# RozDavid/UnScene3D

Measured on AMD Instinct MI355X. Metric: training scenes/sec (Res16UNet34C+Mask3D, 150k voxels), higher is better.
Workload: dtype f32

## Files before the change

unscene3d_amd/csrc/common.h:

```cpp
#pragma once
#include <hip/hip_runtime.h>
#include <stdint.h>
#include <stdio.h>
#include <string.h>

#include "../../include/usc3d.h"

namespace usc {

constexpr int kWave = 64;

void set_error(const char* fmt, ...);

#define USC_REQUIRE(cond, ...)                   \
  do {                                           \
    if (!(cond)) {                               \
      ::usc::set_error(__VA_ARGS__);             \
      return USC_ERR_ARG;                        \
    }                                            \
  } while (0)

#define USC_CHECK_LAUNCH(name)                                                  \
  do {                                                                          \
    hipError_t e__ = hipGetLastError();                                         \
// ... 37 lines not shown
  k ^= k >> 31;
  return k;
}

__host__ __device__ inline int floor_quant(int c, int q) {
  int d = c / q;
  if ((c % q != 0) && ((c < 0) != (q < 0))) --d;
  return d * q;
}

#if defined(__HIPCC__)
__device__ inline int table_lookup(const uint64_t* __restrict__ keys,
                                   const int32_t* __restrict__ vals, int64_t cap,
                                   uint64_t key) {
  uint64_t slot = hash_key(key) & (uint64_t)(cap - 1);
  for (;;) {
    uint64_t k = keys[slot];
    if (k == key) return vals[slot];
    if (k == kEmptyKey) return -1;
    slot = (slot + 1) & (uint64_t)(cap - 1);
  }
}

__device__ inline int lane_id() { return threadIdx.x & 63; }

__device__ inline int wave_reduce_add(int v) {
#pragma unroll
  for (int o = 32; o > 0; o >>= 1) v += __shfl_xor(v, o, 64);
  return v;
}
__device__ inline float wave_reduce_addf(float v) {
#pragma unroll
  for (int o = 32; o > 0; o >>= 1) v += __shfl_xor(v, o, 64);
  return v;
}
__device__ inline double wave_reduce_addd(double v) {
#pragma unroll
  for (int o = 32; o > 0; o >>= 1) v += __shfl_xor(v, o, 64);
  return v;
}
__device__ inline int wave_inclusive_scan(int v) {
  const int l = lane_id();
#pragma unroll
  for (int o = 1; o < 64; o <<= 1) {
    int t = __shfl_up(v, o, 64);
    if (l >= o) v += t;
  }
  return v;
}
#endif

int spconv_up_table(const int32_t* nbr2, int32_t K, int64_t n_coarse, int64_t n_fine, int32_t* inv, hipStream_t st);

}
```

unscene3d_amd/csrc/spconv.hip:

```cpp
#include "common.h"

#include <stdlib.h>

#include <vector>

namespace usc {

typedef float f32x16 __attribute__((ext_vector_type(16)));

#define MFMA32(a, b, c) __builtin_amdgcn_mfma_f32_32x32x2f32((a), (b), (c), 0, 0, 0)

struct GemmParams {
  const float* in;
  const float* W;
  const int32_t* nbr;
  const float* bias;
  float* out;
  int64_t n_out;
  int cin, cout, K;
  int accumulate;
  int G;
  int TM;
  int wt1;
  const int32_t* rows_in;
  const int32_t* rows_out;
  const int64_t* koff;
  unsigned long long* stats;
};

__device__ inline int acc_row(int reg, int half) { return (reg & 3) + 8 * (reg >> 2) + 4 * half; }

template <int NB> struct BVec;
template <> struct BVec<1> { float v[1]; };
template <> struct BVec<2> { float v[2]; };
template <> struct BVec<3> { float v[3]; };
template <> struct BVec<4> { float v[4]; };

template <int NB>
__device__ inline void load_b(const float* __restrict__ p, float (&b)[NB]) {
  if (NB == 4) {
    const float4 t = *reinterpret_cast<const float4*>(p);
    b[0] = t.x; b[1 % NB] = t.y; b[2 % NB] = t.z; b[3 % NB] = t.w;
  } else if (NB == 2) {
    const float2 t = *reinterpret_cast<const float2*>(p);
    b[0] = t.x; b[1 % NB] = t.y;
  } else {
#pragma unroll
    for (int nb = 0; nb < NB; ++nb) b[nb] = p[nb];
  }
}

template <bool LIST>
__device__ inline bool locate_tile(const GemmParams& p, int wave, int i, int& k_begin, int& k_end,
                                   int64_t& my_out_row, int64_t& my_in_row_list) {
  my_out_row = -1;
  my_in_row_list = -1;
// ... 968 lines not shown
  pl.aligned = true;
  const int cb = cout / 32;
  const int cands[4] = {4, 3, 2, 1};
  int chosen = 1;
  for (int c = 0; c < 4; ++c) {
    const int nb = cands[c];
    if (cb % nb) continue;
    if (max_tiles * (cb / nb) >= kTargetWaves) { chosen = nb; break; }
  }
  pl.NB = chosen;
  return pl;
}

template <bool LIST>
static void launch_gemm(const GemmPlan& pl, dim3 grid, hipStream_t st, const GemmParams& p) {
#define USC_GG(NBv)                                                                                      \
  if (pl.aligned && p.wt1)        \
    hipLaunchKernelGGL((gather_gemm_aligned_kernel<NBv, false, true>), grid, dim3(256), 0, st, p);      \
  else if (pl.aligned)                                                                                   \
    hipLaunchKernelGGL((gather_gemm_aligned_kernel<NBv, LIST>), grid, dim3(256), 0, st, p);             \
  else                                                                                                   \
    hipLaunchKernelGGL((gather_gemm_kernel<NBv, LIST>), grid, dim3(256), 0, st, p);
  switch (pl.NB) {
    case 1: USC_GG(1) break;
    case 2: USC_GG(2) break;
    case 3: USC_GG(3) break;
    default: USC_GG(4) break;
  }
#undef USC_GG
}

}

using namespace usc;

extern "C" {

int usc_weight_transpose(const float* W, int32_t K, int32_t cin, int32_t cout, int32_t mirror, float* out,
                         usc_stream_t s) {
  USC_REQUIRE(W && out && K >= 1 && cin >= 1 && cout >= 1, "usc_weight_transpose: bad argument");
  const int64_t total = (int64_t)K * cin * cout;
  hipLaunchKernelGGL(weight_transpose_kernel, dim3(stream_grid(total, 256)), dim3(256), 0, as_stream(s), W, (int)K,
                     (int)cin, (int)cout, (int)mirror, out);
  USC_CHECK_LAUNCH("usc_weight_transpose");
  return USC_OK;
}

int usc_spconv_plan(int32_t kind, int64_t n, int32_t cin, int32_t cout, int32_t K) {
  GemmPlan pl;
  if (kind == 0 && stem_form(K > 1, cin, cout, K)) return 1 | (1 << 14);
  if (kind == 0) pl = plan_table(n, cin, cout, K);
  else if (kind == 1) pl = plan_list(ceil_div(n, 32) + K, cin, cout);
  else {
    const int ctiles = cin / 32, cb = cout / 32;
    const int NBf = (cb % 3 == 0) ? 3 : (cb % 4 == 0 ? 4 : (cb % 2 == 0 ? 2 : 1));
    if (cin % 32 == 0 && cout % 32 == 0 && (!(NBf == 3 && ctiles % 3 != 0) || ctiles % 4 == 0)) {
      const int CT = wgrad_full_ct(ctiles, NBf);
      return NBf | (1 << 8) | (1 << 13) | (CT << 16);
    }
    const int NB = pick_nb(cout);
    pl = GemmPlan{NB, 1, (cin % 32 == 0) && (cout % (NB * 32) == 0), 0};
  }
  return pl.NB | ((pl.aligned ? 1 : 0) << 8) | ((pl.TM > 0 ? 1 : 0) << 12) | (pl.G << 16);
}

int64_t usc_spconv_gather_gemm_ws_bytes(int64_t n_out, int32_t cin, int32_t cout, int32_t K) {
  const GemmPlan pl = plan_table(n_out, cin, cout, K);
  if (pl.TM > 0) return (int64_t)K * cin * cout * 4;
  return pl.G > 1 ? (int64_t)pl.G * n_out * cout * 4 : 0;
}

namespace {
struct LaunchStats { unsigned long long* ring = nullptr; int64_t slots = 0, count = 0; std::vector<usc_launch_stat> meta; };
LaunchStats g_lstats;
__global__ void launch_stats_init_kernel(unsigned long long* ring, int64_t slots) {
  const int64_t i = (int64_t)blockIdx.x * blockDim.x + threadIdx.x;
  if (i < slots) { ring[4 * i] = ~0ull; ring[4 * i + 1] = 0; ring[4 * i + 2] = 0; ring[4 * i + 3] = 0; }
}
}

int usc_launch_stats_begin(void* ring_dev, int64_t slots, usc_stream_t s) {
  USC_REQUIRE(ring_dev && slots > 0, "usc_launch_stats_begin: needs a device ring of slots x 4 x u64");
  hipLaunchKernelGGL(launch_stats_init_kernel, dim3((unsigned)ceil_div(slots, 256)), dim3(256), 0, as_stream(s),
                     (unsigned long long*)ring_dev, slots);
  USC_CHECK_LAUNCH("usc_launch_stats_begin");
  g_lstats.ring = (unsigned long long*)ring_dev;
  g_lstats.slots = slots;
  g_lstats.count = 0;
  g_lstats.meta.clear();
  g_lstats.meta.reserve((size_t)slots);
  return USC_OK;
}

int64_t usc_launch_stats_end(usc_launch_stat* host_out, int64_t max_out) {
  const int64_t n = g_lstats.count;
  if (host_out)
    for (int64_t i = 0; i < n && i < max_out; ++i) host_out[i] = g_lstats.meta[(size_t)i];
  g_lstats.ring = nullptr;
  g_lstats.slots = g_lstats.count = 0;
  g_lstats.meta.clear();
  return n;
}

int64_t usc_wall_clock_khz(void) {
  int dev = 0, khz = 0;
  if (hipGetDevice(&dev) != hipSuccess || hipDeviceGetAttribute(&khz, hipDeviceAttributeWallClockRate, dev) != hipSuccess) return 0;
  return khz;
}

int usc_spconv_gather_gemm(const float* in, int64_t n_in, int32_t cin, const float* W, int32_t K, int32_t cout,
                           const int32_t* nbr, int64_t n_out, const float* bias, float* out, int32_t accumulate,
                           int32_t w_transposed, void* ws, int64_t ws_bytes, usc_stream_t s) {
  USC_REQUIRE(cin >= 1 && cout >= 1 && K >= 1 && n_out >= 0 && n_in >= 0, "usc_spconv_gather_gemm: bad sizes");
  USC_REQUIRE(nbr || K == 1, "usc_spconv_gather_gemm: K>1 needs a neighbour table");
  USC_REQUIRE(nbr || n_in == n_out, "usc_spconv_gather_gemm: identity map needs n_in == n_out");
  if (n_out == 0) return USC_OK;
  USC_REQUIRE(in && W && out, "usc_spconv_gather_gemm: null pointer");
  if (stem_form(nbr != nullptr, cin, cout, K) && !accumulate && !w_transposed) {
    hipLaunchKernelGGL(stem_conv_kernel, dim3((unsigned)ceil_div(n_out, 256)), dim3(256), 0, as_stream(s), in, W, nbr, bias,
                       out, n_out, (int)K, (int)cin);
    USC_CHECK_LAUNCH("usc_spconv_gather_gemm");
    return USC_OK;
  }
  const GemmPlan pl = plan_table(n_out, cin, cout, K);
  GemmParams p{};
  p.in = in; p.W = W; p.nbr = nbr; p.bias = bias; p.out = out;
  p.n_out = n_out; p.cin = cin; p.cout = cout; p.K = K; p.accumulate = accumulate; p.G = pl.G;
  if (pl.G > 1) {
    USC_REQUIRE(ws && ws_bytes >= (int64_t)pl.G * n_out * cout * 4, "usc_spconv_gather_gemm: workspace too small");
    p.out = (float*)ws;
  }
  hipStream_t st = as_stream(s);
  const bool wt1 = w_transposed && K == 1 && !nbr && pl.aligned && pl.TM == 0;
  USC_REQUIRE(!w_transposed || pl.TM > 0 || wt1,
              "usc_spconv_gather_gemm: w_transposed is only folded into the tile-compacted kernel (usc_spconv_plan bit 12) "
              "and, for K = 1 on identity rows with channel counts in multiples of 32, into the row-order kernel; "
              "use usc_weight_transpose for other shapes");
  p.wt1 = wt1 ? 1 : 0;
  if (pl.TM > 0) {
    p.TM = pl.TM;
    USC_REQUIRE(ws && ws_bytes >= (int64_t)K * cin * cout * 4, "usc_spconv_gather_gemm: workspace too small");
    hipLaunchKernelGGL(weight_pack_kernel, dim3(stream_grid((int64_t)K * cin * cout, 256)), dim3(256), 0, st, W, (int)K,
                       (int)cin, (int)cout, pl.NB, (int)w_transposed, (float*)ws);
    p.W = (const float*)ws;
    dim3 cgrid((unsigned)ceil_div(n_out, pl.TM), (unsigned)(cout / (pl.NB * 32)));
    const size_t lds = compact_lds_bytes(pl.NB, pl.TM);
    if (g_lstats.ring && g_lstats.count < g_lstats.slots) {
      p.stats = g_lstats.ring + 4 * g_lstats.count++;
      g_lstats.meta.push_back(usc_launch_stat{n_out, cin, cout, K, pl.NB});
    }
#define USC_CG(NBv)                                                                                        \
    {                                                                                                      \
      static bool attr_set = false;                                                                        \
      auto kfn = gather_gemm_compact_kernel<NBv>;                                                          \
      if (!attr_set) {                                                                                     \
        (void)hipFuncSetAttribute((const void*)kfn, hipFuncAttributeMaxDynamicSharedMemorySize, 160 * 1024); \
        attr_set = true;                                                                                   \
      }                                                                                                    \
      hipLaunchKernelGGL(kfn, cgrid, dim3(64 * kCompactWaves), lds, st, p);                                \
    }
    if (pl.NB == 3) USC_CG(3) else if (pl.NB == 2) USC_CG(2) else USC_CG(1)
#undef USC_CG
    USC_CHECK_LAUNCH("usc_spconv_gather_gemm");
    return USC_OK;
  }
  dim3 grid((unsigned)ceil_div(n_out, 128), (unsigned)ceil_div(cout, pl.NB * 32), (unsigned)pl.G);
  launch_gemm<false>(pl, grid, st, p);
  if (pl.G > 1) {
    const int64_t numel4 = n_out * cout / 4;
    hipLaunchKernelGGL(group_reduce_kernel, dim3(stream_grid(numel4, 256)), dim3(256), 0, st, (const float*)ws, pl.G,
                       numel4, (int)cout, bias, (int)accumulate, out);
  }
  USC_CHECK_LAUNCH("usc_spconv_gather_gemm");
  return USC_OK;
}

int usc_spconv_pairs_gemm(const float* in, int32_t cin, const float* W, int32_t K, int32_t cout,
                          const int32_t* rows_in, const int32_t* rows_out, const int64_t* koff, int64_t P_capacity,
                          float* out, usc_stream_t s) {
  USC_REQUIRE(cin >= 1 && cout >= 1 && K >= 1 && P_capacity >= 0, "usc_spconv_pairs_gemm: bad sizes");
  if (P_capacity == 0) return USC_OK;
  USC_REQUIRE(in && W && rows_in && rows_out && koff && out, "usc_spconv_pairs_gemm: null pointer");
  GemmParams p{};
  p.in = in; p.W = W; p.out = out; p.cin = cin; p.cout = cout; p.K = K; p.G = 1;
  p.rows_in = rows_in; p.rows_out = rows_out; p.koff = koff;
  const int64_t max_tiles = ceil_div(P_capacity, 32) + K;
  const GemmPlan pl = plan_list(max_tiles, cin, cout);
  dim3 grid((unsigned)ceil_div(max_tiles, 4), (unsigned)ceil_div(cout, pl.NB * 32));
  launch_gemm<true>(pl, grid, as_stream(s), p);
  USC_CHECK_LAUNCH("usc_spconv_pairs_gemm");
  return USC_OK;
}

int64_t usc_spconv_wgrad_ws_bytes(int32_t K, int32_t cin, int32_t cout) {
  return (int64_t)64 * K * cin * cout * (int64_t)sizeof(float);
}

int64_t usc_spconv_wgrad_ws_bytes_rows(int32_t K, int32_t cin, int32_t cout, int64_t n_rows) {
  const int64_t numel = (int64_t)K * cin * cout;
  const int ctiles = cin / 32, cb = cout / 32;
  if (cin % 32 == 0 && cout % 32 == 0 && cb > 0) {
    const int NBf = wgrad_full_nb(cb);
    if (!(NBf == 3 && ctiles % 3 != 0) || ctiles % 4 == 0)
      return wgrad_full_splits(K, ctiles, cb, wgrad_full_ct(ctiles, NBf), NBf, n_rows) * numel * 4;
  }
  return (int64_t)wgrad_splits(K, cin, cout, pick_nb(cout), n_rows) * numel * 4;
}

int64_t usc_spconv_wgrad_table_ws_bytes(int32_t K, int32_t cin, int32_t cout) {
  return (int64_t)kStemSplits * K * cin * cout * 4;
}

int usc_spconv_wgrad_table(const float* in, int32_t cin, const float* dy, int32_t cout, const int32_t* nbr, int32_t K,
                           int64_t n_out, float* dW, int32_t accumulate, void* ws, int64_t ws_bytes, usc_stream_t s) {
  USC_REQUIRE(cin >= 1 && cin <= 4 && cout == 32 && K >= 1 && K <= 32 && n_out >= 0,
              "usc_spconv_wgrad_table: the table form covers <= 4 input channels and 32 output channels (the stem)");
  USC_REQUIRE(in && dy && nbr && dW && ws, "usc_spconv_wgrad_table: null pointer");
  USC_REQUIRE(ws_bytes >= usc_spconv_wgrad_table_ws_bytes(K, cin, cout), "usc_spconv_wgrad_table: workspace too small");
  hipStream_t st = as_stream(s);
  const int per = 32 / cin, groups = (K + per - 1) / per;
  const int64_t numel = (int64_t)K * cin * 32;
  hipLaunchKernelGGL(stem_wgrad_kernel, dim3(kStemSplits, (unsigned)groups), dim3(64 * kStemWaves), 0, st, in, dy, nbr, n_out, (int)K,
                     (int)cin, (float*)ws);
  hipLaunchKernelGGL(wgrad_reduce_kernel, dim3(stream_grid(numel, 256)), dim3(256), 0, st, (const float*)ws, kStemSplits, numel,
                     (int)accumulate, dW);
  USC_CHECK_LAUNCH("usc_spconv_wgrad_table");
  return USC_OK;
}

static int g_wgrad_grid_limit = 0;
void usc_spconv_wgrad_grid_limit(int32_t max_workgroups) { g_wgrad_grid_limit = max_workgroups; }

int usc_spconv_wgrad(const float* a, int32_t cin, const float* b, int32_t cout, int32_t K, const int32_t* a_idx,
                     const int32_t* b_idx, const int64_t* koff, int64_t n_rows, float* dW, int32_t accumulate, void* ws, int64_t ws_bytes,
                     usc_stream_t s) {
  USC_REQUIRE(cin >= 1 && cout >= 1 && K >= 1 && n_rows >= 0, "usc_spconv_wgrad: bad sizes");
  USC_REQUIRE(a && b && dW && ws, "usc_spconv_wgrad: null pointer");
  USC_REQUIRE((a_idx && b_idx && koff) || (!a_idx && K == 1), "usc_spconv_wgrad: pair lists required for K>1");
  const int64_t numel = (int64_t)K * cin * cout;
  hipStream_t st = as_stream(s);
  WgradParams p{};
  p.a = a; p.b = b; p.a_idx = a_idx; p.b_idx = b_idx; p.koff = koff; p.n_rows = n_rows;
  p.partial = (float*)ws; p.cin = cin; p.cout = cout; p.K = K;
  const int ctiles = cin / 32, cb = cout / 32;
  const int NBf = wgrad_full_nb(cb);
  if (cin % 32 == 0 && cout % 32 == 0 && (!(NBf == 3 && ctiles % 3 != 0) || ctiles % 4 == 0)) {
    const int CT = wgrad_full_ct(ctiles, NBf);
    const int64_t S = wgrad_full_splits(K, ctiles, cb, CT, NBf, n_rows);
    USC_REQUIRE(ws_bytes >= S * numel * 4, "usc_spconv_wgrad: workspace too small");
    p.S = (int)S;
    if (S == 1) { p.direct = dW; p.accumulate = accumulate; }
    dim3 grid((unsigned)(K * S), (unsigned)(ctiles / CT), (unsigned)(cb / NBf));
    if (g_wgrad_grid_limit > 0 && (int64_t)K * S > g_wgrad_grid_limit) {
      p.vblocks = (int)(K * S);
      grid.x = (unsigned)g_wgrad_grid_limit;
    }
    const size_t lds = (size_t)4 * NBf * 16 * 64 * sizeof(float);
#define USC_WF(C, N) if (CT == C && NBf == N) { \
      static bool attr_set = false; auto kfn = wgrad_full_kernel<C, N>; \
      if (!attr_set) { (void)hipFuncSetAttribute((const void*)kfn, hipFuncAttributeMaxDynamicSharedMemorySize, 64 * 1024); attr_set = true; } \
      hipLaunchKernelGGL(kfn, grid, dim3(256), lds, st, p, WgradGroup{}); }
    USC_WF(3, 3) USC_WF(2, 3) USC_WF(1, 3) USC_WF(2, 4) USC_WF(1, 4) USC_WF(4, 2) USC_WF(3, 2) USC_WF(2, 2) USC_WF(1, 2) USC_WF(4, 1) USC_WF(3, 1) USC_WF(2, 1) USC_WF(1, 1)
    USC_WF(4, 3)
#undef USC_WF
    if (S > 1)
      hipLaunchKernelGGL(wgrad_reduce_kernel, dim3(stream_grid(numel, 256)), dim3(256), 0, st, (const float*)ws, (int)S,
                         numel, (int)accumulate, dW);
    USC_CHECK_LAUNCH("usc_spconv_wgrad");
    return USC_OK;
  }
  const int NB = pick_nb(cout);
  const bool aligned = (cin % 32 == 0) && (cout % (NB * 32) == 0);
  const int S = wgrad_splits(K, cin, cout, NB, n_rows);
  USC_REQUIRE(ws_bytes >= (int64_t)S * numel * 4, "usc_spconv_wgrad: workspace too small");
  p.S = S;
  dim3 grid((unsigned)(K * S), (unsigned)ceil_div(cin, 32), (unsigned)ceil_div(cout, NB * 32));
  const size_t lds = (size_t)3 * NB * 16 * 64 * sizeof(float);
#define USC_WG(NBv)                                                                          \
  if (aligned) hipLaunchKernelGGL((wgrad_kernel<NBv, true>), grid, dim3(256), lds, st, p);  \
  else hipLaunchKernelGGL((wgrad_kernel<NBv, false>), grid, dim3(256), lds, st, p);
  switch (NB) {
    case 1: USC_WG(1) break;
    case 2: USC_WG(2) break;
    case 3: USC_WG(3) break;
    default: USC_WG(4) break;
  }
#undef USC_WG
  hipLaunchKernelGGL(wgrad_reduce_kernel, dim3(stream_grid(numel, 256)), dim3(256), 0, st, (const float*)ws, S, numel,
                     (int)accumulate, dW);
  USC_CHECK_LAUNCH("usc_spconv_wgrad");
  return USC_OK;
}

int32_t usc_spconv_wgrad_group_max(void) { return kMaxWgradGroup; }

int usc_spconv_wgrad_group_ok(int32_t R, int32_t cin, int32_t cout, int32_t K, int64_t n_rows) {
// ... 46 lines not shown
```

unscene3d_amd/ops.py:

```python
from __future__ import annotations

from dataclasses import dataclass

import ctypes
import os

import torch

from . import profiler as _prof
from ._lib import check, lib, require_device


def _stream():
    return torch._C._cuda_getCurrentRawStream(torch._C._cuda_getDevice())


def _chk(t: torch.Tensor, dtype, name: str):
    if not isinstance(t, torch.Tensor):
        raise RuntimeError(f"{name} must be a torch.Tensor")
    if not t.is_cuda:
        raise RuntimeError(f"{name} must be a HIP (cuda) tensor — unscene3d_amd has no CPU path")
    if t.dtype != dtype:
        raise RuntimeError(f"{name} must be {dtype}, got {t.dtype}")
    if not t.is_contiguous():
# ... 83 lines not shown
def kernel_map_cube(cmap: CoordMap, ksize: int = 3) -> torch.Tensor:
    K = ksize ** 3
    nbr = torch.empty((K, cmap.n), dtype=torch.int32, device=cmap.coords.device)
    check(lib.usc_kernel_map_cube(_ptr(cmap.coords), cmap.n, cmap.tensor_stride, ksize, _ptr(cmap.table_keys),
                                  _ptr(cmap.table_vals), cmap.cap, _ptr(nbr), _stream()), "usc_kernel_map_cube")
    return nbr


def kernel_map_down2(fine: CoordMap, parent: torch.Tensor, coarse: CoordMap):
    dev = fine.coords.device
    nbr2 = torch.full((8, coarse.n), -1, dtype=torch.int32, device=dev)
    kidx = torch.empty(fine.n, dtype=torch.uint8, device=dev)
    check(lib.usc_kernel_map_down2(_ptr(fine.coords), fine.n, fine.tensor_stride, _ptr(parent), _ptr(coarse.coords),
                                   coarse.n, _ptr(nbr2), _ptr(kidx), _stream()), "usc_kernel_map_down2")
    return nbr2, kidx


class Rulebook:

    def __init__(self, in_idx, out_idx, koff, capacity, P=None):
        self.in_idx, self.out_idx, self.koff, self.capacity = in_idx, out_idx, koff, capacity
        self._P = P

    @property
    def P(self) -> int:
        if self._P is None:
            self._P = int(self.koff[-1].item())
        return self._P


def rulebook_compact(nbr: torch.Tensor) -> Rulebook:
    _chk(nbr, torch.int32, "nbr")
    K, n_out = nbr.shape
    dev = nbr.device
    in_idx = torch.empty(K * n_out, dtype=torch.int32, device=dev)
    out_idx = torch.empty(K * n_out, dtype=torch.int32, device=dev)
    koff = torch.empty(K + 1, dtype=torch.int64, device=dev)
    ws = _ws(lib.usc_rulebook_ws_bytes(K, n_out), dev)
    check(lib.usc_rulebook_compact(_ptr(nbr), K, n_out, _ptr(in_idx), _ptr(out_idx), _ptr(koff), _ptr(ws),
                                   ws.numel(), _stream()), "usc_rulebook_compact")
    return Rulebook(in_idx, out_idx, koff, K * n_out)


def _conv_cost(P, n_in, n_out, K, cin, cout):
    return 2.0 * P * cin * cout, 4.0 * (n_in * cin + n_out * cout + K * cin * cout) + 8.0 * P


def _sorted_symbol(cout):
    cb = cout // 32
    nb = 4 if cb % 4 == 0 else 3 if cb % 3 == 0 else 2 if cb % 2 == 0 else 1
    return f"usc::gather_gemm_sorted_kernel<{nb}, {4 if nb == 4 else 8}>"


def _kernel_symbol(kind, n, cin, cout, K):
    code = lib.usc_spconv_plan(kind, int(n), cin, cout, K)
    nb, aligned, compact = code & 0xFF, (code >> 8) & 1, (code >> 12) & 1
    tag = f" [n={int(n)} cin={cin} cout={cout} K={K} G={code >> 16}]" if _prof.SHAPES else ""
    if kind == 0 and (code >> 14) & 1:
        return "usc::stem_conv_kernel" + tag
    if kind == 0 and compact:
        return f"usc::gather_gemm_compact_kernel<{nb}>" + tag
    if kind == 2:
        if (code >> 13) & 1:
            return f"usc::wgrad_full_kernel<{code >> 16}, {nb}>" + tag
        return f"usc::wgrad_kernel<{nb}, {'true' if aligned else 'false'}>" + tag
    base = "usc::gather_gemm_aligned_kernel" if aligned else "usc::gather_gemm_kernel"
    return f"{base}<{nb}, {'true' if kind == 1 else 'false'}>" + tag


def weight_transpose(W: torch.Tensor, mirror: bool) -> torch.Tensor:
    _chk(W, torch.float32, "W")
    K, cin, cout = W.shape
    out = torch.empty((K, cout, cin), dtype=torch.float32, device=W.device)
    check(lib.usc_weight_transpose(_ptr(W), K, cin, cout, int(mirror), _ptr(out), _stream()), "usc_weight_transpose")
    return out


def rowsort(nbr: torch.Tensor):
    cached = getattr(nbr, "_usc_rowsort", None)
    if cached is not None:
        return cached
    _chk(nbr, torch.int32, "nbr")
    K, n_out = nbr.shape
    dev = nbr.device
    perm = torch.empty(n_out, dtype=torch.int32, device=dev)
    tmask = torch.empty((n_out + 31) // 32, dtype=torch.int32, device=dev)
    ws = _ws(lib.usc_rowsort_ws_bytes(K, n_out), dev)
    check(lib.usc_rowsort_build(_ptr(nbr), K, n_out, _ptr(perm), _ptr(tmask), _ptr(ws), ws.numel(), _stream()),
          "usc_rowsort_build")
    nbr._usc_rowsort = (perm, tmask)
    return perm, tmask


CONV_PATH = os.environ.get("USC3D_CONV", "sorted")


def _sorted_applies(nbr, K, cin, cout):
    if CONV_PATH == "legacy" or nbr is None or not (1 < K <= 32) or cin % 32 or cout % 32 or cin > 4096:
        return False
    if CONV_PATH == "sorted-all":
        return True
    compact = (lib.usc_spconv_plan(0, int(nbr.shape[1]), cin, cout, K) >> 12) & 1
    return not compact


def gather_gemm(feats, W, nbr, n_out, bias=None, out=None, accumulate=False, w_transposed=False):
    _chk(feats, torch.float32, "feats")
    _chk(W, torch.float32, "W")
    if w_transposed:
        K, cout, cin = W.shape
        linear_form = nbr is None and K == 1 and cin % 32 == 0 and cout % 32 == 0
        if not (linear_form or _sorted_applies(nbr, K, cin, cout) or
                (nbr is not None and (lib.usc_spconv_plan(0, int(n_out), cin, cout, K) >> 12) & 1)):
            W = weight_transpose(W, mirror=K > 1)
            w_transposed = False
    K, cin, cout = (W.shape[0], W.shape[2], W.shape[1]) if w_transposed else W.shape
    if feats.shape[1] != cin:
        raise RuntimeError(f"gather_gemm: feats have {feats.shape[1]} channels, kernel expects {cin}")
    if nbr is not None:
        _chk(nbr, torch.int32, "nbr")
        if nbr.shape[0] != K or nbr.shape[1] != n_out:
            raise RuntimeError("gather_gemm: neighbour table shape mismatch")
    if out is None:
        out = torch.empty((n_out, cout), dtype=torch.float32, device=feats.device)
    if bias is not None:
        _chk(bias, torch.float32, "bias")
    if _sorted_applies(nbr, K, cin, cout):
        perm, tmask = rowsort(nbr)
        wsb = lib.usc_spconv_sorted_ws_bytes(n_out, cin, cout, K)
        ws = _ws(wsb, feats.device) if wsb > 0 else None
        with _prof.maybe(lambda: _sorted_symbol(cout) + (f" [n={n_out} cin={cin} cout={cout} K={K}]" if _prof.SHAPES else ""),
                         lambda: _conv_cost(_prof.table_pairs(nbr), feats.shape[0], n_out, K, cin, cout)):
            check(lib.usc_spconv_sorted_gemm(_ptr(feats), feats.shape[0], cin, _ptr(W), K, cout, _ptr(nbr), _ptr(perm),
                                             _ptr(tmask), n_out, _ptr(bias), _ptr(out), int(accumulate),
                                             int(w_transposed), _ptr(ws), wsb, _stream()), "usc_spconv_sorted_gemm")
        return out
    wsb = lib.usc_spconv_gather_gemm_ws_bytes(n_out, cin, cout, K)
    ws = _ws(wsb, feats.device) if wsb > 0 else None
    with _prof.maybe(lambda: _kernel_symbol(0, n_out, cin, cout, K),
                     lambda: _conv_cost(_prof.table_pairs(nbr) if nbr is not None else n_out, feats.shape[0], n_out,
                                        K, cin, cout)):
        check(lib.usc_spconv_gather_gemm(_ptr(feats), feats.shape[0], cin, _ptr(W), K, cout, _ptr(nbr), n_out,
                                         _ptr(bias), _ptr(out), int(accumulate), int(w_transposed), _ptr(ws), wsb,
                                         _stream()), "usc_spconv_gather_gemm")
    return out


def cast_bf16(x: torch.Tensor) -> torch.Tensor:
    _chk(x, torch.float32, "x")
    out = torch.empty(x.shape, dtype=torch.bfloat16, device=x.device)
    check(lib.usc_cast_bf16(_ptr(x), x.numel(), _ptr(out), _stream()), "usc_cast_bf16")
    return out


def _gather_gemm_planes(xs, planes, cin, Wp, K, cout, nbr, n_out, bias, out, accumulate):
    if planes is None:
        name, ws_bytes, gemm, split = "usc_spconv_gather_gemm_bf16", lib.usc_spconv_gather_gemm_bf16_ws_bytes, \
            lib.usc_spconv_gather_gemm_bf16, ()
    else:
        name, ws_bytes, gemm, split = "usc_spconv_gather_gemm_split", lib.usc_spconv_gather_gemm_split_ws_bytes, \
            lib.usc_spconv_gather_gemm_split, (planes,)
    if nbr is not None:
        _chk(nbr, torch.int32, "nbr")
        if nbr.shape[0] != K or nbr.shape[1] != n_out:
            raise RuntimeError(f"{name[11:]}: neighbour table shape mismatch")
    if out is None:
        out = torch.empty((n_out, cout), dtype=torch.float32, device=xs.device)
    if bias is not None:
        _chk(bias, torch.float32, "bias")
    wsb = ws_bytes(n_out, cin, cout, K, *split)
    ws = _ws(wsb, xs.device) if wsb > 0 else None
    check(gemm(_ptr(xs), xs.shape[0], cin, _ptr(Wp), K, cout, *split, _ptr(nbr), n_out, _ptr(bias), _ptr(out),
               int(accumulate), _ptr(ws), max(wsb, 0), _stream()), name)
    return out


def gather_gemm_bf16(feats, Wp, K, cout, nbr, n_out, bias=None, out=None, accumulate=False):
    if feats.dtype == torch.float32:
        feats = cast_bf16(feats.contiguous())
    _chk(feats, torch.bfloat16, "feats")
    _chk(Wp, torch.bfloat16, "Wp")
    cin = feats.shape[1]
    if Wp.numel() != K * cin * cout:
        raise RuntimeError("gather_gemm_bf16: packed weights do not match K, cin, cout")
    return _gather_gemm_planes(feats, None, cin, Wp, K, cout, nbr, n_out, bias, out, accumulate)


def split_bf16(x: torch.Tensor, planes: int) -> torch.Tensor:
    _chk(x, torch.float32, "x")
    if x.dim() == 1:
        out = torch.empty((planes, x.shape[0]), dtype=torch.bfloat16, device=x.device)
        check(lib.usc_split_bf16(_ptr(x), x.numel(), planes, _ptr(out), _stream()), "usc_split_bf16")
# ... 72 lines not shown
def _graph_task():
    return torch._C._current_graph_task_id()


def _join_after_backward():
    global _JOIN_QUEUED_TASK
    if not SIDE_STREAMS or not on_side_stream():
        return
    task = _graph_task()
    if task < 0 or task == _JOIN_QUEUED_TASK:
        return
    _JOIN_QUEUED_TASK = task

    def done():
        global _JOIN_QUEUED_TASK
        _JOIN_QUEUED_TASK = None
        join_side_streams()
    torch.autograd.Variable._execution_engine.queue_callback(done)


PARAMS_FINAL_HOOK = None


def _params_final(params):
    if PARAMS_FINAL_HOOK is not None and params:
        PARAMS_FINAL_HOOK(params)


def _grad_written(*params):
    _join_after_backward()
    if GRAD_WRITTEN_HOOK is not None:
        for p in params:
            if p is not None:
                GRAD_WRITTEN_HOOK(p)


def wgrad(a, b, K, a_idx=None, b_idx=None, koff=None, into=None, out=None, nbr=None):
    _chk(a, torch.float32, "a")
    _chk(b, torch.float32, "b")
    cin, cout = a.shape[1], b.shape[1]
    dW = into if into is not None else (out if out is not None else
                                        torch.empty((K, cin, cout), dtype=torch.float32, device=a.device))
    if nbr is not None and cin <= 4 and cout == 32 and K <= 32 and nbr.shape == (K, b.shape[0]):
        wsb = lib.usc_spconv_wgrad_table_ws_bytes(K, cin, cout)
        ws = _ws(wsb, a.device)
        with _prof.maybe(lambda: "usc::stem_wgrad_kernel" + (f" [n={b.shape[0]} cin={cin} cout={cout} K={K}]" if _prof.SHAPES else ""),
                         lambda: _conv_cost(_prof.table_pairs(nbr), a.shape[0], b.shape[0], K, cin, cout)):
            check(lib.usc_spconv_wgrad_table(_ptr(a), cin, _ptr(b), cout, _ptr(nbr), K, b.shape[0], _ptr(dW),
                                             int(into is not None), _ptr(ws), ws.numel(), _stream()),
                  "usc_spconv_wgrad_table")
        return dW
    ws = _ws(lib.usc_spconv_wgrad_ws_bytes(K, cin, cout), a.device)
    n_rows = a.shape[0] if a_idx is None else int(a_idx.shape[0])
    with _prof.maybe(lambda: _kernel_symbol(2, n_rows, cin, cout, K),
                     lambda: _conv_cost(n_rows if koff is None else int(koff[-1].item()), a.shape[0], b.shape[0], K,
                                        cin, cout)):
        check(lib.usc_spconv_wgrad(_ptr(a), cin, _ptr(b), cout, K, _ptr(a_idx), _ptr(b_idx), _ptr(koff), n_rows,
                                   _ptr(dW), int(into is not None), _ptr(ws), ws.numel(), _stream()), "usc_spconv_wgrad")
    return dW


def wgrad_group(a_list, b_list, into_list, K, a_idx, b_idx, koff):
    import ctypes as C
    R = len(a_list)
    if not (R == len(b_list) == len(into_list) and 1 <= R <= lib.usc_spconv_wgrad_group_max()):
        raise RuntimeError("wgrad_group: between 1 and usc_spconv_wgrad_group_max() problems, three lists of equal length")
    cin, cout = a_list[0].shape[1], b_list[0].shape[1]
    for a, b, w in zip(a_list, b_list, into_list):
        _chk(a, torch.float32, "a")
        _chk(b, torch.float32, "b")
        _chk(w, torch.float32, "dW")
        if a.shape[1] != cin or b.shape[1] != cout or w.numel() != K * cin * cout:
            raise RuntimeError("wgrad_group: the problems of a group have one shape")
    n_rows = a_list[0].shape[0] if a_idx is None else int(a_idx.shape[0])
    pa = (C.c_void_p * R)(*[t.data_ptr() for t in a_list])
    pb = (C.c_void_p * R)(*[t.data_ptr() for t in b_list])
    pw = (C.c_void_p * R)(*[t.data_ptr() for t in into_list])
    check(lib.usc_spconv_wgrad_group(R, pa, pb, pw, cin, cout, K, _ptr(a_idx), _ptr(b_idx), _ptr(koff), n_rows, 1,
                                     _stream()), "usc_spconv_wgrad_group")
    return into_list


class _ConvSame(torch.autograd.Function):

    @staticmethod
    def forward(ctx, feats, W, bias, nbr, get_rulebook):
        feats = feats.contiguous()
        W3 = W if W.dim() == 3 else W[None]
        out = gather_gemm(feats, W3.contiguous(), nbr, feats.shape[0], bias=None if bias is None else bias.reshape(-1))
        ctx.save_for_backward(feats, W3)
        ctx.nbr, ctx.get_rulebook = nbr, get_rulebook
        ctx.w_dim, ctx.has_bias = W.dim(), bias is not None
        ctx.w_param = W
        return out

    @staticmethod
    def backward(ctx, dout):
        feats, W3 = ctx.saved_tensors
        dout = dout.contiguous()
        K = W3.shape[0]
        dfeats = dW = dbias = None
        if ctx.needs_input_grad[0]:
            if K > 1:
                dfeats = gather_gemm(dout, W3.contiguous(), ctx.nbr, feats.shape[0], w_transposed=True)
            else:
                dfeats = gather_gemm(dout, weight_transpose(W3.contiguous(), mirror=False), ctx.nbr, feats.shape[0])
        if ctx.needs_input_grad[1]:
# ... 1067 lines not shown
```

Baseline: 43.83.

## Add dense MFMA kernels for identity 1x1 sparse conv forward and weight gradient

Routes K==1 convolutions that have no neighbour table to new dense kernels. The forward kernel keeps the whole weight matrix in LDS and streams contiguous row tiles through MFMA. The weight-gradient kernel reduces over row chunks with double-buffered LDS staging and split-row partials that a separate reduce step sums. Both skip the gather and index machinery the generic sparse paths use for these layers. The cost is new alignment and workspace requirements, and extra partial buffers for the split reduction.

```diff
diff --git a/unscene3d_amd/csrc/common.h b/unscene3d_amd/csrc/common.h
--- a/unscene3d_amd/csrc/common.h
+++ b/unscene3d_amd/csrc/common.h
@@ -113,4 +113,14 @@
 
 int spconv_up_table(const int32_t* nbr2, int32_t K, int64_t n_coarse, int64_t n_fine, int32_t* inv, hipStream_t st);
 
+constexpr int64_t kDenseWgradRows = 8192, kDenseWgradRows128 = 1024, kDenseWgradRowsWide = 16384, kDenseRowsMin = 24576;
+constexpr int kDenseRowsMinCin = 64, kDenseRowsMaxWBytes = 64 * 1024;
+bool dense_wgrad_routed(int64_t n_rows, int cin, int cout);
+int dense_wgrad_splits(int64_t n_rows, int cin, int cout);
+void dense_wgrad_launch(const float* x, const float* dy, int64_t n, int cin, int cout, int S, float* dst, int rmw,
+                        hipStream_t st);
+bool dense_rows_routed(int64_t n, int cin, int cout);
+void dense_rows_launch(const float* x, const float* W, const float* bias, float* out, int64_t n, int cin, int cout, int wt,
+                       int accumulate, hipStream_t st);
+
 }
diff --git a/unscene3d_amd/csrc/dense.hip b/unscene3d_amd/csrc/dense.hip
--- /dev/null
+++ b/unscene3d_amd/csrc/dense.hip
@@ -0,0 +1,301 @@
+#include "common.h"
+
+namespace usc {
+
+typedef float f32x16 __attribute__((ext_vector_type(16)));
+
+#define MFMA32(a, b, c) __builtin_amdgcn_mfma_f32_32x32x2f32((a), (b), (c), 0, 0, 0)
+
+__device__ inline int dense_acc_row(int reg, int half) { return (reg & 3) + 8 * (reg >> 2) + 4 * half; }
+
+constexpr int kDwChunk = 64;
+
+struct DenseWgradParams {
+  const float* x;
+  const float* dy;
+  float* dst;
+  int64_t n;
+  int cin, cout, S;
+  int ctiles;
+  int tiles;
+  int rmw;
+};
+
+template <int NB>
+__global__ __launch_bounds__(256, NB == 4 ? 1 : 2) void dense_wgrad_kernel(DenseWgradParams p) {
+  constexpr int BN = NB * 32;
+  constexpr int XV = kDwChunk * 32 / 4 / 256, YV = kDwChunk * BN / 4 / 256;
+  constexpr int kTile = kDwChunk * (32 + BN);
+  constexpr int kLds = kTile > 4 * 16 * 64 ? kTile : 4 * 16 * 64;
+  __shared__ __attribute__((aligned(16))) float lds[kLds];
+  float* const xs = lds;
+  float* const ys = lds + kDwChunk * 32;
+  const int tid = threadIdx.x, lane = tid & 63, wave = tid >> 6;
+  const int i = lane & 31, h = lane >> 5;
+  const int L = blockIdx.x;
+  const int slab = (L / (8 * p.tiles)) * 8 + (L & 7);
+  const int tile = (L >> 3) % p.tiles;
+  if (slab >= p.S) return;
+  const int ci0 = (tile % p.ctiles) * 32, co0 = (tile / p.ctiles) * BN;
+  const int cin = p.cin, cout = p.cout;
+  const int64_t chunks = (p.n + kDwChunk - 1) / kDwChunk;
+  const int64_t c_begin = (int64_t)slab * chunks / p.S, c_end = (int64_t)(slab + 1) * chunks / p.S;
+
+  f32x16 acc[NB];
+#pragma unroll
+  for (int nb = 0; nb < NB; ++nb)
+#pragma unroll
+    for (int r = 0; r < 16; ++r) acc[nb][r] = 0.f;
+
+  struct Stage { float4 x[XV]; float4 y[YV]; };
+  auto gload = [&](Stage& st, int64_t chunk) __attribute__((always_inline)) {
+    const int64_t r0 = chunk * kDwChunk, last = p.n - 1;
+#pragma unroll
+    for (int u = 0; u < XV; ++u) {
+      const int e = tid + 256 * u, row = e >> 3, c4 = e & 7;
+      const int64_t r = r0 + row < last ? r0 + row : last;
+      st.x[u] = *reinterpret_cast<const float4*>(p.x + r * (int64_t)cin + ci0 + 4 * c4);
+    }
+#pragma unroll
+    for (int u = 0; u < YV; ++u) {
+      const int e = tid + 256 * u, row = e / (8 * NB), c4 = e - row * (8 * NB);
+      const int64_t r = r0 + row < last ? r0 + row : last;
+      st.y[u] = *reinterpret_cast<const float4*>(p.dy + r * (int64_t)cout + co0 + 4 * c4);
+    }
+  };
+  auto lstore = [&](const Stage& st, int64_t chunk) __attribute__((always_inline)) {
+    const int64_t r0 = chunk * kDwChunk;
+#pragma unroll
+    for (int u = 0; u < XV; ++u) {
+      const int e = tid + 256 * u;
+      const float keep = r0 + (e >> 3) < p.n ? 1.f : 0.f;
+      const float4 v = st.x[u];
+      reinterpret_cast<float4*>(xs)[e] = keep != 0.f ? v : make_float4(0.f, 0.f, 0.f, 0.f);
+    }
+#pragma unroll
+    for (int u = 0; u < YV; ++u) {
+      const int e = tid + 256 * u;
+      const float keep = r0 + e / (8 * NB) < p.n ? 1.f : 0.f;
+      const float4 v = st.y[u];
+      reinterpret_cast<float4*>(ys)[e] = keep != 0.f ? v : make_float4(0.f, 0.f, 0.f, 0.f);
+    }
+  };
+  auto compute = [&]() __attribute__((always_inline)) {
+    const float* xa = xs + (16 * wave + h) * 32 + i;
+    const float* yb = ys + (16 * wave + h) * BN + i;
+#pragma unroll
+    for (int s = 0; s < 8; ++s) {
+      const float a = xa[2 * s * 32];
+      float b[NB];
+#pragma unroll
+      for (int nb = 0; nb < NB; ++nb) b[nb] = yb[2 * s * BN + nb * 32];
+#pragma unroll
+      for (int nb = 0; nb < NB; ++nb) acc[nb] = MFMA32(a, b[nb], acc[nb]);
+    }
+  };
+  Stage sa, sb;
+  gload(sa, c_begin);
+  gload(sb, c_begin + 1);
+  if (c_begin < c_end) lstore(sa, c_begin);
+  __syncthreads();
+  for (int64_t c = c_begin; c < c_end; c += 2) {
+    gload(sa, c + 2);
+    compute();
+    __syncthreads();
+    if (c + 1 >= c_end) break;
+    lstore(sb, c + 1);
+    __syncthreads();
+    gload(sb, c + 3);
+    compute();
+    __syncthreads();
+    if (c + 2 < c_end) lstore(sa, c + 2);
+    __syncthreads();
+  }
+
+  float* dst = p.dst + (p.S > 1 ? (int64_t)slab * cin * cout : 0);
+#pragma unroll
+  for (int nb = 0; nb < NB; ++nb) {
+    if (nb) __syncthreads();
+#pragma unroll
+    for (int r = 0; r < 16; ++r) lds[(wave * 16 + r) * 64 + lane] = acc[nb][r];
+    __syncthreads();
+#pragma unroll
+    for (int rr = 0; rr < 4; ++rr) {
+      const int r = 4 * wave + rr;
+      float t = lds[(3 * 16 + r) * 64 + lane];
+      t += lds[(2 * 16 + r) * 64 + lane];
+      t += lds[(1 * 16 + r) * 64 + lane];
+      const float v = lds[r * 64 + lane] + t;
+      float* o = dst + (int64_t)(ci0 + dense_acc_row(r, h)) * cout + co0 + nb * 32 + i;
+      *o = p.rmw ? *o + v : v;
+    }
+  }
+}
+
+static int dense_wgrad_nb(int cb) { return cb % 4 == 0 ? 4 : (cb % 3 == 0 ? 3 : (cb % 2 == 0 ? 2 : 1)); }
+
+bool dense_wgrad_routed(int64_t n_rows, int cin, int cout) {
+  if (cin < 32 || cout < 32 || cin % 32 || cout % 32) return false;
+  return n_rows >= (cin == 128 ? kDenseWgradRows128 : (cin < 128 ? kDenseWgradRows : kDenseWgradRowsWide));
+}
+
+int dense_wgrad_splits(int64_t n_rows, int cin, int cout) {
+  const int cb = cout / 32;
+  const int64_t tiles = (int64_t)(cin / 32) * (cb / dense_wgrad_nb(cb));
+  int64_t S = (512 + tiles / 2) / tiles;
+  const int64_t by_rows = n_rows / 256;
+  if (S > by_rows) S = by_rows;
+  if (S > 64) S = 64;
+  if (S < 1) S = 1;
+  return (int)S;
+}
+
+void dense_wgrad_launch(const float* x, const float* dy, int64_t n, int cin, int cout, int S, float* dst, int rmw,
+                        hipStream_t st) {
+  const int cb = cout / 32, NB = dense_wgrad_nb(cb);
+  DenseWgradParams p{};
+  p.x = x; p.dy = dy; p.dst = dst; p.n = n; p.cin = cin; p.cout = cout; p.S = S;
+  p.ctiles = cin / 32; p.tiles = p.ctiles * (cb / NB); p.rmw = rmw;
+  const dim3 grid((unsigned)(ceil_div(S, 8) * 8 * p.tiles));
+  switch (NB) {
+    case 1: hipLaunchKernelGGL(dense_wgrad_kernel<1>, grid, dim3(256), 0, st, p); break;
+    case 2: hipLaunchKernelGGL(dense_wgrad_kernel<2>, grid, dim3(256), 0, st, p); break;
+    case 3: hipLaunchKernelGGL(dense_wgrad_kernel<3>, grid, dim3(256), 0, st, p); break;
+    default: hipLaunchKernelGGL(dense_wgrad_kernel<4>, grid, dim3(256), 0, st, p); break;
+  }
+}
+
+struct DenseRowsParams {
+  const float* x;
+  const float* W;
+  const float* bias;
+  float* out;
+  int64_t n;
+  int cin, cout, wt, accumulate;
+};
+
+template <int NB>
+__global__ __launch_bounds__(256, 2) void dense_rows_kernel(DenseRowsParams p) {
+  extern __shared__ __attribute__((aligned(16))) float ws_lds[];
+  const int tid = threadIdx.x, lane = tid & 63, wave = tid >> 6;
+  const int i = lane & 31, h = lane >> 5;
+  const int cin = p.cin, cout = p.cout;
+  const bool w16 = (reinterpret_cast<uintptr_t>(p.W) & 15) == 0;
+  if (!p.wt) {
+    if (w16) {
+      for (int e = tid; e < cin * cout / 4; e += 256)
+        reinterpret_cast<float4*>(ws_lds)[e] = reinterpret_cast<const float4*>(p.W)[e];
+    } else {
+      for (int e = tid; e < cin * cout; e += 256) ws_lds[e] = p.W[e];
+    }
+  } else {
+    for (int e = tid; e < cout * (cin / 4); e += 256) {
+      const int c4 = e / cout, n = e - c4 * cout;
+      const float* src = p.W + (int64_t)n * cin + 4 * c4;
+      float w[4];
+      if (w16) {
+        const float4 t = *reinterpret_cast<const float4*>(src);
+        w[0] = t.x; w[1] = t.y; w[2] = t.z; w[3] = t.w;
+      } else {
+#pragma unroll
+        for (int j = 0; j < 4; ++j) w[j] = src[j];
+      }
+#pragma unroll
+      for (int j = 0; j < 4; ++j) ws_lds[(4 * c4 + j) * cout + n] = w[j];
+    }
+  }
+  __syncthreads();
+
+  const int64_t tiles = (p.n + 31) / 32;
+  const int64_t nw = (int64_t)gridDim.x * 4;
+  int64_t tile = (int64_t)blockIdx.x * 4 + wave;
+  if (tile >= tiles) return;
+  auto row_ptr = [&](int64_t t) __attribute__((always_inline)) -> const float* {
+    int64_t r = t * 32 + i;
+    if (r >= p.n) r = p.n - 1;
+    return p.x + r * (int64_t)cin + 4 * h;
+  };
+  const float* ar = row_ptr(tile);
+  float4 a[4];
+#pragma unroll
+  for (int t = 0; t < 4; ++t) a[t] = *reinterpret_cast<const float4*>(ar + 8 * t);
+  for (; tile < tiles; tile += nw) {
+    f32x16 acc[NB];
+#pragma unroll
+    for (int nb = 0; nb < NB; ++nb)
+#pragma unroll
+      for (int r = 0; r < 16; ++r) acc[nb][r] = 0.f;
+    const float* ar_next = row_ptr(tile + nw < tiles ? tile + nw : tile);
+    for (int c0 = 0; c0 < cin; c0 += 32) {
+      const float* nx = c0 + 32 < cin ? ar + c0 + 32 : ar_next;
+      float4 an[4];
+#pragma unroll
+      for (int t = 0; t < 4; ++t) an[t] = *reinterpret_cast<const float4*>(nx + 8 * t);
+#pragma unroll
+      for (int t = 0; t < 4; ++t) {
+        const float av[4] = {a[t].x, a[t].y, a[t].z, a[t].w};
+#pragma unroll
+        for (int j = 0; j < 4; ++j) {
+          const float* wrow = ws_lds + (c0 + 8 * t + 4 * h + j) * cout + i;
+          float b[NB];
+#pragma unroll
+          for (int nb = 0; nb < NB; ++nb) b[nb] = wrow[nb * 32];
+#pragma unroll
+          for (int nb = 0; nb < NB; ++nb) acc[nb] = MFMA32(av[j], b[nb], acc[nb]);
+        }
+      }
+#pragma unroll
+      for (int t = 0; t < 4; ++t) a[t] = an[t];
+    }
+    float bv[NB];
+#pragma unroll
+    for (int nb = 0; nb < NB; ++nb) bv[nb] = p.bias ? p.bias[nb * 32 + i] : 0.f;
+#pragma unroll
+    for (int r = 0; r < 16; ++r) {
+      const int64_t orow = tile * 32 + dense_acc_row(r, h);
+      if (orow >= p.n) continue;
+      float* dst = p.out + orow * (int64_t)cout + i;
+#pragma unroll
+      for (int nb = 0; nb < NB; ++nb) {
+        float v = acc[nb][r];
+        if (p.bias) v += bv[nb];
+        if (p.accumulate) v += dst[nb * 32];
+        dst[nb * 32] = v;
+      }
+    }
+    ar = ar_next;
+  }
+}
+
+bool dense_rows_routed(int64_t n, int cin, int cout) {
+  if (cin % 32 || cout % 32 || cout < 32 || cout > 128) return false;
+  return n >= kDenseRowsMin && cin >= kDenseRowsMinCin && (int64_t)cin * cout * 4 <= kDenseRowsMaxWBytes;
+}
+
+void dense_rows_launch(const float* x, const float* W, const float* bias, float* out, int64_t n, int cin, int cout,
+                       int wt, int accumulate, hipStream_t st) {
+  DenseRowsParams p{};
+  p.x = x; p.W = W; p.bias = bias; p.out = out; p.n = n; p.cin = cin; p.cout = cout; p.wt = wt; p.accumulate = accumulate;
+  int64_t wgs = ceil_div(ceil_div(n, 32), 4);
+  if (wgs > 512) wgs = 512;
+  const size_t lds = (size_t)cin * cout * sizeof(float);
+#define USC_DR(N)                                                                                              \
+  {                                                                                                            \
+    static bool attr_set = false;                                                                              \
+    auto kfn = dense_rows_kernel<N>;                                                                           \
+    if (!attr_set) {                                                                                           \
+      (void)hipFuncSetAttribute((const void*)kfn, hipFuncAttributeMaxDynamicSharedMemorySize, 64 * 1024);      \
+      attr_set = true;                                                                                         \
+    }                                                                                                          \
+    hipLaunchKernelGGL(kfn, dim3((unsigned)wgs), dim3(256), lds, st, p);                                       \
+  }
+  switch (cout / 32) {
+    case 1: USC_DR(1) break;
+    case 2: USC_DR(2) break;
+    case 3: USC_DR(3) break;
+    default: USC_DR(4) break;
+  }
+#undef USC_DR
+}
+
+}
diff --git a/unscene3d_amd/csrc/spconv.hip b/unscene3d_amd/csrc/spconv.hip
--- a/unscene3d_amd/csrc/spconv.hip
+++ b/unscene3d_amd/csrc/spconv.hip
@@ -2,6 +2,7 @@
 
 #include <stdlib.h>
 
+#include <algorithm>
 #include <vector>
 
 namespace usc {
@@ -1076,16 +1077,19 @@
   if (kind == 0) pl = plan_table(n, cin, cout, K);
   else if (kind == 1) pl = plan_list(ceil_div(n, 32) + K, cin, cout);
   else {
+    const int dense = (K == 1 && dense_wgrad_routed(n, cin, cout)) ? (1 << 15) : 0;
     const int ctiles = cin / 32, cb = cout / 32;
     const int NBf = (cb % 3 == 0) ? 3 : (cb % 4 == 0 ? 4 : (cb % 2 == 0 ? 2 : 1));
     if (cin % 32 == 0 && cout % 32 == 0 && (!(NBf == 3 && ctiles % 3 != 0) || ctiles % 4 == 0)) {
       const int CT = wgrad_full_ct(ctiles, NBf);
-      return NBf | (1 << 8) | (1 << 13) | (CT << 16);
+      return NBf | (1 << 8) | (1 << 13) | dense | (CT << 16);
     }
     const int NB = pick_nb(cout);
     pl = GemmPlan{NB, 1, (cin % 32 == 0) && (cout % (NB * 32) == 0), 0};
-  }
-  return pl.NB | ((pl.aligned ? 1 : 0) << 8) | ((pl.TM > 0 ? 1 : 0) << 12) | (pl.G << 16);
+    return pl.NB | ((pl.aligned ? 1 : 0) << 8) | dense | (pl.G << 16);
+  }
+  const int dense = (kind == 0 && K == 1 && dense_rows_routed(n, cin, cout)) ? (1 << 15) : 0;
+  return pl.NB | ((pl.aligned ? 1 : 0) << 8) | ((pl.TM > 0 ? 1 : 0) << 12) | dense | (pl.G << 16);
 }
 
 int64_t usc_spconv_gather_gemm_ws_bytes(int64_t n_out, int32_t cin, int32_t cout, int32_t K) {
@@ -1143,6 +1147,12 @@
   if (stem_form(nbr != nullptr, cin, cout, K) && !accumulate && !w_transposed) {
     hipLaunchKernelGGL(stem_conv_kernel, dim3((unsigned)ceil_div(n_out, 256)), dim3(256), 0, as_stream(s), in, W, nbr, bias,
                        out, n_out, (int)K, (int)cin);
+    USC_CHECK_LAUNCH("usc_spconv_gather_gemm");
+    return USC_OK;
+  }
+  if (!nbr && K == 1 && dense_rows_routed(n_out, cin, cout)) {
+    USC_REQUIRE((reinterpret_cast<uintptr_t>(in) & 15) == 0, "usc_spconv_gather_gemm: `in` must be 16-byte aligned");
+    dense_rows_launch(in, W, bias, out, n_out, cin, cout, w_transposed ? 1 : 0, accumulate ? 1 : 0, as_stream(s));
     USC_CHECK_LAUNCH("usc_spconv_gather_gemm");
     return USC_OK;
   }
@@ -1223,12 +1233,14 @@
 int64_t usc_spconv_wgrad_ws_bytes_rows(int32_t K, int32_t cin, int32_t cout, int64_t n_rows) {
   const int64_t numel = (int64_t)K * cin * cout;
   const int ctiles = cin / 32, cb = cout / 32;
+  int64_t dense = 0;
+  if (K == 1 && dense_wgrad_routed(n_rows, cin, cout)) dense = (int64_t)dense_wgrad_splits(n_rows, cin, cout) * numel * 4;
   if (cin % 32 == 0 && cout % 32 == 0 && cb > 0) {
     const int NBf = wgrad_full_nb(cb);
     if (!(NBf == 3 && ctiles % 3 != 0) || ctiles % 4 == 0)
-      return wgrad_full_splits(K, ctiles, cb, wgrad_full_ct(ctiles, NBf), NBf, n_rows) * numel * 4;
-  }
-  return (int64_t)wgrad_splits(K, cin, cout, pick_nb(cout), n_rows) * numel * 4;
+      return std::max(dense, wgrad_full_splits(K, ctiles, cb, wgrad_full_ct(ctiles, NBf), NBf, n_rows) * numel * 4);
+  }
+  return std::max(dense, (int64_t)wgrad_splits(K, cin, cout, pick_nb(cout), n_rows) * numel * 4);
 }
 
 int64_t usc_spconv_wgrad_table_ws_bytes(int32_t K, int32_t cin, int32_t cout) {
@@ -1266,6 +1278,18 @@
   WgradParams p{};
   p.a = a; p.b = b; p.a_idx = a_idx; p.b_idx = b_idx; p.koff = koff; p.n_rows = n_rows;
   p.partial = (float*)ws; p.cin = cin; p.cout = cout; p.K = K;
+  if (!a_idx && K == 1 && dense_wgrad_routed(n_rows, cin, cout)) {
+    USC_REQUIRE(((reinterpret_cast<uintptr_t>(a) | reinterpret_cast<uintptr_t>(b)) & 15) == 0,
+                "usc_spconv_wgrad: `a` and `b` must be 16-byte aligned");
+    const int S = dense_wgrad_splits(n_rows, cin, cout);
+    USC_REQUIRE(S == 1 || ws_bytes >= (int64_t)S * numel * 4, "usc_spconv_wgrad: workspace too small");
+    dense_wgrad_launch(a, b, n_rows, cin, cout, S, S == 1 ? dW : (float*)ws, S == 1 && accumulate, st);
+    if (S > 1)
+      hipLaunchKernelGGL(wgrad_reduce_kernel, dim3(stream_grid(numel, 256)), dim3(256), 0, st, (const float*)ws, S, numel,
+                         (int)accumulate, dW);
+    USC_CHECK_LAUNCH("usc_spconv_wgrad");
+    return USC_OK;
+  }
   const int ctiles = cin / 32, cb = cout / 32;
   const int NBf = wgrad_full_nb(cb);
   if (cin % 32 == 0 && cout % 32 == 0 && (!(NBf == 3 && ctiles % 3 != 0) || ctiles % 4 == 0)) {
diff --git a/unscene3d_amd/ops.py b/unscene3d_amd/ops.py
--- a/unscene3d_amd/ops.py
+++ b/unscene3d_amd/ops.py
@@ -159,10 +159,15 @@
     return f"usc::gather_gemm_sorted_kernel<{nb}, {4 if nb == 4 else 8}>"
 
 
-def _kernel_symbol(kind, n, cin, cout, K):
+def _kernel_symbol(kind, n, cin, cout, K, identity=False):
     code = lib.usc_spconv_plan(kind, int(n), cin, cout, K)
     nb, aligned, compact = code & 0xFF, (code >> 8) & 1, (code >> 12) & 1
     tag = f" [n={int(n)} cin={cin} cout={cout} K={K} G={code >> 16}]" if _prof.SHAPES else ""
+    if identity and (code >> 15) & 1:
+        cb = cout // 32
+        if kind == 2:
+            return f"usc::dense_wgrad_kernel<{4 if cb % 4 == 0 else 3 if cb % 3 == 0 else 2 if cb % 2 == 0 else 1}>" + tag
+        return f"usc::dense_rows_kernel<{cb}>" + tag
     if kind == 0 and (code >> 14) & 1:
         return "usc::stem_conv_kernel" + tag
     if kind == 0 and compact:
@@ -244,7 +249,7 @@
         return out
     wsb = lib.usc_spconv_gather_gemm_ws_bytes(n_out, cin, cout, K)
     ws = _ws(wsb, feats.device) if wsb > 0 else None
-    with _prof.maybe(lambda: _kernel_symbol(0, n_out, cin, cout, K),
+    with _prof.maybe(lambda: _kernel_symbol(0, n_out, cin, cout, K, identity=nbr is None),
                      lambda: _conv_cost(_prof.table_pairs(nbr) if nbr is not None else n_out, feats.shape[0], n_out,
                                         K, cin, cout)):
         check(lib.usc_spconv_gather_gemm(_ptr(feats), feats.shape[0], cin, _ptr(W), K, cout, _ptr(nbr), n_out,
@@ -423,7 +428,7 @@
         return dW
     ws = _ws(lib.usc_spconv_wgrad_ws_bytes(K, cin, cout), a.device)
     n_rows = a.shape[0] if a_idx is None else int(a_idx.shape[0])
-    with _prof.maybe(lambda: _kernel_symbol(2, n_rows, cin, cout, K),
+    with _prof.maybe(lambda: _kernel_symbol(2, n_rows, cin, cout, K, identity=a_idx is None),
                      lambda: _conv_cost(n_rows if koff is None else int(koff[-1].item()), a.shape[0], b.shape[0], K,
                                         cin, cout)):
         check(lib.usc_spconv_wgrad(_ptr(a), cin, _ptr(b), cout, K, _ptr(a_idx), _ptr(b_idx), _ptr(koff), n_rows,
```

New measurement: 43.83, median of 5. About the same (-0.0%).
